# SamSweere/xmm-superres-denoise

Measured on NVIDIA B200. Metric: RRDB SR-2x inference images/sec (F=32, nb=4, 416x416 -> 832x832, batch 64 per GPU), higher is better.
Workload: dtype bf16

## Files before the change

xmm_superres_denoise_b200/csrc/conv3x3_rdb.cuh:

```cuda
#pragma once
#include <cstdio>

#include "conv3x3_tc.cuh"

namespace xmm {

constexpr int kRdbP = 63;
constexpr int kRdbBoxPx = kRdbP + 2;
constexpr int kRdbTileData = 2 * kRdbBoxPx * 64;
constexpr int kRdbTileBytes = 17 * 512;
constexpr int kRdbThreads = 512;
constexpr int kRdbSlots = 5;
constexpr int kRdbSlotCols = kRdbSlots * 32;
constexpr int kRdbMaxRing = 8;
constexpr int kRdbMaxStages = 16;
template <bool PAIR>
constexpr int kRdbLRing = PAIR ? kRdbMaxStages : 8;
constexpr int kRdbTapBytes = 32 * 64;
constexpr int kRdbGroupBytes = 3 * kRdbTapBytes;
constexpr int kRdbProfSlots = 24;

struct RdbLayerArgs {
  const void* wblob;
  uint32_t w_bytes;
  uint32_t smem_off;
  float lrelu_slope;
  int store;
  __nv_bfloat16* out;
  int out_ctot, out_coff;
};

struct RdbArgs {
  RdbLayerArgs layer[3];
  int cin_off;
  int batch, height, width, band_h, tiles_x;
  long long total_rows;
  int stages, ring0, ring1;
  uint32_t w_total;
  float s0, s1, s2;
  const __nv_bfloat16* r1;
  int r1_ctot, r1_coff;
  const __nv_bfloat16* r2;
  int r2_ctot, r2_coff;
  int backoff_ns;
  int prefetch_rows;
  int split_producers;
  long long* prof;
};

template <int NL>
__host__ __device__ inline int rdb_tile_origin(int t) {
  return t == 0 ? 0 : (kRdbP - (NL - 1)) + (t - 1) * (kRdbP - 2 * (NL - 1));
}
template <int NL>
__host__ __device__ inline int rdb_tiles_x(int width) {
  int n = 1;
  while ((n == 1 ? 0 : rdb_tile_origin<NL>(n - 1) - (NL - 1)) + kRdbP < width) ++n;
  return n;
}

struct RdbPiece {
  int b, x0;
  int own_lo, own_hi;
  int ra, rb;
};

template <int NL, bool PAIR = false>
struct RdbSched {
  int band_h, tiles_x, width, c0, npieces;
  int ncols, rank;
  long long t0, t1;
  __device__ __forceinline__ void init(const RdbArgs& a) {
    band_h = a.band_h;
    tiles_x = a.tiles_x;
    width = a.width;
    if (PAIR) {
      ncols = a.batch * a.tiles_x;
      rank = int(ptx::cluster_ctarank());
      const long long unit = blockIdx.x >> 1, nunits = gridDim.x >> 1;
      t0 = a.total_rows * unit / nunits;
      t1 = a.total_rows * (unit + 1) / nunits;
    } else {
      t0 = a.total_rows * blockIdx.x / gridDim.x;
      t1 = a.total_rows * (blockIdx.x + 1) / gridDim.x;
    }
    c0 = int(t0 / band_h);
    npieces = t1 > t0 ? int((t1 - 1) / band_h) - c0 + 1 : 0;
  }
  __device__ __forceinline__ RdbPiece get(int i) const {
    RdbPiece p;
    int col = c0 + i;
    const long long base = (long long)col * band_h;
    p.ra = t0 > base ? int(t0 - base) : 0;
    p.rb = t1 < base + band_h ? int(t1 - base) : band_h;
    bool phantom = false;
    if (PAIR) {
      col = 2 * col + rank;
      phantom = col >= ncols;
      if (phantom) col = ncols - 1;
    }
    p.b = col / tiles_x;
    const int t = col - p.b * tiles_x;
    p.own_lo = rdb_tile_origin<NL>(t);
    p.x0 = t == 0 ? 0 : p.own_lo - (NL - 1);
    p.own_hi = phantom ? p.own_lo : t == tiles_x - 1 ? width : rdb_tile_origin<NL>(t + 1);
    return p;
  }
};

template <int NL, class S, class F>
__device__ __forceinline__ void rdb_walk(const S& s, F&& f) {
  int piece[NL], r[NL], hi[NL], n[NL], seq[NL][NL];
  RdbPiece pc[NL];
  bool done[NL];
#pragma unroll
  for (int l = 0; l < NL; ++l) {
    piece[l] = 0;
    n[l] = 0;
    done[l] = s.npieces == 0;
#pragma unroll
    for (int m = 0; m < NL; ++m) seq[l][m] = 0;
    pc[l] = s.get(0);
    r[l] = pc[l].ra - (NL - 1 - l) - 1;
    hi[l] = pc[l].rb + (NL - 1 - l) + 2;
  }
  while (!done[NL - 1]) {
    uint32_t go = done[0] ? 0u : 1u;
    bool steady = !done[0];
    int reps = pc[0].rb + (NL - 1) - r[0] + 1;
#pragma unroll
    for (int l = 1; l < NL; ++l) {
      const bool ready = !done[l] && (done[l - 1] || piece[l - 1] > piece[l] || (piece[l - 1] == piece[l] && r[l - 1] > r[l] + 1));
      go |= ready ? (1u << l) : 0u;
      steady = steady && ready && piece[l] == piece[0];
      const int kl = pc[l].rb + (NL - 1 - l) - r[l] + 1;
      reps = kl < reps ? kl : reps;
    }
    if (!steady || reps < 1) reps = 1;
    for (int i = 0; i < reps; ++i) {
#pragma unroll
      for (int l = 0; l < NL; ++l) {
        if ((go >> l) & 1u) {
          const int e = NL - 1 - l;
          f(l, pc[l], r[l], r[l] > pc[l].rb + e, n[l], seq[l]);
          ++n[l];
          if (++r[l] > hi[l]) {
#pragma unroll
            for (int m = 0; m < NL; ++m) seq[l][m] += (pc[l].rb - pc[l].ra) + 2 * (NL - 1 - m);
            if (++piece[l] >= s.npieces) {
              done[l] = true;
            } else {
              pc[l] = s.get(piece[l]);
              r[l] = pc[l].ra - e - 1;
              hi[l] = pc[l].rb + e + 2;
            }
          }
        }
      }
    }
  }
}

__device__ __noinline__ void rdb_wait_timeout(int tag, int a, int b2, int c) {
  printf("conv3x3_rdb: CTA %d thread %d stuck in wait %d (layer/map %d, index %d, parity %d)\n", int(blockIdx.x),
         int(threadIdx.x), tag, a, b2, c);
  __trap();
}
__device__ __forceinline__ void rdb_wait(uint64_t* bar, uint32_t parity, int tag, int a, int b2) {
  uint32_t spins = 0;
  while (!ptx::mbar_try_wait(bar, parity)) {
    if (++spins > (1u << 26)) rdb_wait_timeout(tag, a, b2, int(parity));
  }
}

__device__ __forceinline__ void rdb_wait_backoff(uint64_t* bar, uint32_t parity, int tag, int a, int b2, uint32_t ns) {
  uint32_t spins = 0;
  while (!ptx::mbar_try_wait(bar, parity)) {
    if (ns) __nanosleep(ns);
    if (++spins > (1u << 24)) rdb_wait_timeout(tag, a, b2, int(parity));
  }
}
#ifndef XMM_RDB_PROFILE
#define XMM_RDB_PROFILE 0
#endif
__device__ __forceinline__ void rdb_wait_p(uint64_t* bar, uint32_t parity, int tag, int a, int b2, bool prof, long long& acc) {
  if (XMM_RDB_PROFILE && prof) {
    const long long t0 = clock64();
    rdb_wait(bar, parity, tag, a, b2);
    acc += clock64() - t0;
  } else {
    rdb_wait(bar, parity, tag, a, b2);
  }
}

__device__ __forceinline__ int rdb_phi(int row) { return (row + 30) % 3; }

__device__ __forceinline__ void tmem_st_zero32(uint32_t taddr) {
  const uint32_t z = 0;
  asm volatile(
      "tcgen05.st.sync.aligned.32x32b.x32.b32 [%0], "
      "{%1, %1, %1, %1, %1, %1, %1, %1, %1, %1, %1, %1, %1, %1, %1, %1, "
      "%1, %1, %1, %1, %1, %1, %1, %1, %1, %1, %1, %1, %1, %1, %1, %1};" ::"r"(taddr),
      "r"(z)
      : "memory");
}
__device__ __forceinline__ void tmem_st_32x32(uint32_t taddr, const uint32_t (&r)[32]) {
  asm volatile(
      "tcgen05.st.sync.aligned.32x32b.x32.b32 [%0], "
      "{%1, %2, %3, %4, %5, %6, %7, %8, %9, %10, %11, %12, %13, %14, %15, %16, "
      "%17, %18, %19, %20, %21, %22, %23, %24, %25, %26, %27, %28, %29, %30, %31, %32};" ::"r"(taddr),
      "r"(r[0]), "r"(r[1]), "r"(r[2]), "r"(r[3]), "r"(r[4]), "r"(r[5]), "r"(r[6]), "r"(r[7]), "r"(r[8]), "r"(r[9]), "r"(r[10]),
      "r"(r[11]), "r"(r[12]), "r"(r[13]), "r"(r[14]), "r"(r[15]), "r"(r[16]), "r"(r[17]), "r"(r[18]), "r"(r[19]), "r"(r[20]),
      "r"(r[21]), "r"(r[22]), "r"(r[23]), "r"(r[24]), "r"(r[25]), "r"(r[26]), "r"(r[27]), "r"(r[28]), "r"(r[29]), "r"(r[30]),
      "r"(r[31])
      : "memory");
}
__device__ __forceinline__ void st_global_256(void* p, const uint4& a, const uint4& b) {
  asm volatile("st.global.v8.b32 [%0], {%1, %2, %3, %4, %5, %6, %7, %8};" ::"l"(p), "r"(a.x), "r"(a.y), "r"(a.z), "r"(a.w),
               "r"(b.x), "r"(b.y), "r"(b.z), "r"(b.w)
               : "memory");
}
__device__ __forceinline__ void ld_global_nc_256(const void* p, uint4& a, uint4& b) {
  asm volatile("ld.global.nc.v8.b32 {%0, %1, %2, %3, %4, %5, %6, %7}, [%8];"
               : "=r"(a.x), "=r"(a.y), "=r"(a.z), "=r"(a.w), "=r"(b.x), "=r"(b.y), "=r"(b.z), "=r"(b.w)
               : "l"(p));
}
__device__ __forceinline__ void tmem_st_wait() { asm volatile("tcgen05.wait::st.sync.aligned;" ::: "memory"); }

struct RdbCtx {
  uint8_t* w_s;
  uint8_t* stage_s;
  uint8_t* map_s[2];
  uint64_t* lfull;
  uint64_t* empty;
  uint64_t* tfull;
  uint64_t* tdrain;
  uint64_t* mfull;
  uint64_t* mempty;
  uint64_t* w_bar;
  volatile int* lstage;
  uint32_t tmem_base;
};

template <int G, int NL, int L, bool PAIR>
__device__ __forceinline__ void rdb_issuer(const RdbArgs& args, const RdbCtx& c, const RdbSched<NL, PAIR>& sched) {
  constexpr int NM = NL - 1;
  constexpr int e = NL - 1 - L;
  constexpr int ring[2] = {NL == 3 ? 5 : 2, 3};
  constexpr uint32_t kR = kRdbLRing<PAIR>;
  rdb_wait(c.w_bar, 0, 7, L, 0);
  ptx::tc_fence_after();
  const uint64_t bdesc0 = ptx::umma_smem_desc(ptx::smem_u32(c.w_s), 16, 512, ptx::UMMA_SW64);
  const uint64_t adesc0 = ptx::umma_smem_desc(ptx::smem_u32(c.stage_s), 16, 512, ptx::UMMA_SW64);
  const uint32_t a_hi = uint32_t(adesc0 >> 32), b_hi = uint32_t(bdesc0 >> 32);
  const uint32_t a_lo0 = uint32_t(adesc0);
  const uint32_t b_l = uint32_t(bdesc0) + (args.layer[L].smem_off >> 4);
  const uint32_t a_map0[2] = {a_lo0 + uint32_t((c.map_s[0] - c.stage_s) >> 4), a_lo0 + uint32_t((c.map_s[1] - c.stage_s) >> 4)};
  constexpr uint32_t kTile16 = uint32_t(kRdbTileBytes) >> 4;
  constexpr uint32_t kGroup16 = uint32_t(PAIR ? kRdbGroupBytes / 2 : kRdbGroupBytes) >> 4;
  constexpr uint32_t kChunk16 = 3 * kGroup16;
  constexpr uint32_t kIdesc = ptx::umma_idesc_bf16_f32(PAIR ? 256 : 128, 96, 0, 0);
  auto issue6 = [&](uint32_t d, uint32_t a, uint32_t b) {
#pragma unroll
    for (int dx = 0; dx < 3; ++dx)
#pragma unroll
      for (int ks = 0; ks < 2; ++ks) {
        const uint32_t a_lo = a + uint32_t((dx * 64 + ks * 32) >> 4), b_lo = b + uint32_t(dx) * kGroup16 + uint32_t((ks * 32) >> 4);
        if constexpr (PAIR)
          ptx::umma_ss_lh_pair<true>(d, a_lo, a_hi, b_lo, b_hi, kIdesc);
        else
          ptx::umma_ss_lh<true>(d, a_lo, a_hi, b_lo, b_hi, kIdesc);
      }
  };
  auto commit = [](uint64_t* bar) {
    if constexpr (PAIR)
      ptx::umma_commit_pair(bar);
    else
      ptx::umma_commit(bar);
  };
  const bool prof = XMM_RDB_PROFILE && args.prof != nullptr && L == 0;
  long long pw[3] = {0, 0, 0};
  const long long t_begin = XMM_RDB_PROFILE ? clock64() : 0;
  uint32_t fills = 0;
  uint32_t n = 0;
  int seq[2] = {0, 0};
  for (int pi = 0; pi < sched.npieces; ++pi) {
    const RdbPiece pc = sched.get(pi);
    const int r_last = pc.rb + e;
    for (int r = pc.ra - e - 1; r <= r_last + 2; ++r, ++n) {
      if (n > 0) rdb_wait_p(&c.tdrain[L], (n - 1u) & 1u, 2, L, int(n), prof, pw[0]);
      ptx::tc_fence_after();
      if (r <= r_last) {
        const uint32_t d = c.tmem_base + uint32_t(L * kRdbSlotCols + rdb_phi(r - 1) * 32);
        auto global_chunks = [&]() {
#pragma unroll
          for (int g = 0; g < G; ++g) {
            const int k = int(fills % kR);
            rdb_wait_p(&c.lfull[L * kR + k], (fills / kR) & 1u, 3, L, k, prof, pw[1]);
            const int stage = c.lstage[L * kR + k];
            ++fills;
            ptx::tc_fence_after();
            issue6(d, a_lo0 + uint32_t(stage) * kTile16, b_l + uint32_t(g) * kChunk16);
            commit(&c.empty[stage]);
          }
        };
        auto map_chunks = [&]() {
#pragma unroll
          for (int m = 0; m < NM; ++m)
            if (m < L) {
              const int sq = seq[m] + (r - (pc.ra - (NL - 1 - m)));
              const int slot = sq % ring[m];
              rdb_wait_p(&c.mfull[m * 8 + slot], uint32_t(sq / ring[m]) & 1u, 4, L * 10 + m, sq, prof, pw[2]);
              ptx::tc_fence_after();
              issue6(d, a_map0[m] + uint32_t(slot) * kTile16, b_l + uint32_t(G + m) * kChunk16);
              if (L == NL - 1 || r < pc.ra - e || r > pc.rb + e - 1) commit(&c.mempty[m * 8 + slot]);
            }
        };
        if (NL == 2) {
          map_chunks();
          global_chunks();
        } else {
          global_chunks();
          map_chunks();
        }
      }
      commit(&c.tfull[L]);
    }
#pragma unroll
    for (int m = 0; m < NM; ++m) seq[m] += (pc.rb - pc.ra) + 2 * (NL - 1 - m);
  }
  if (XMM_RDB_PROFILE && prof) {
    long long* o = args.prof + size_t(blockIdx.x) * kRdbProfSlots;
    o[0] = clock64() - t_begin;
    o[1] = pw[0];
    o[2] = pw[1];
    o[3] = pw[2];
  }
}

template <int G, int NL, int L, bool PAIR>
__device__ __forceinline__ void rdb_epilogue(const RdbArgs& args, const RdbCtx& c, const RdbSched<NL, PAIR>& sched, int q,
                                             int lane) {
  const bool remote = PAIR && sched.rank != 0;
  auto arrive = [&](uint64_t* bar) {
    if (remote)
      ptx::mbar_arrive_cluster(ptx::mapa(ptx::smem_u32(bar), 0));
    else
      ptx::mbar_arrive(bar);
  };
  constexpr int e = NL - 1 - L;
  constexpr int ring[2] = {NL == 3 ? 5 : 2, 3};
  constexpr bool last = L == NL - 1;
  const int pos = q * 32 + lane + 1;
  const int band = pos >= kRdbBoxPx ? 1 : 0;
  const int pl = band ? pos - (kRdbBoxPx + 1) : pos - 1;
  const bool lane_ok = band ? pl >= 0 : pl < kRdbP;
  const uint32_t lane_base = c.tmem_base + (uint32_t(q * 32) << 16) + uint32_t(L * kRdbSlotCols);
  const uint32_t pos_off = uint32_t(pos) * 64u;
  const uint32_t pos_xor = uint32_t(pos >> 1) & 3u;
  const uint32_t bias_a = ptx::smem_u32(c.w_s + args.layer[L].smem_off + args.layer[L].w_bytes);
  const float slope = args.layer[L].lrelu_slope;
  const bool has_r1 = last && args.r1 != nullptr, has_r2 = last && args.r2 != nullptr;
  const bool prof = XMM_RDB_PROFILE && args.prof != nullptr;
  long long pw[2] = {0, 0};
  long long ph[4] = {0, 0, 0, 0};
  long long tph = 0;
  const long long t_begin = XMM_RDB_PROFILE ? clock64() : 0;
  uint32_t n = 0;
  int seq = 0;
  for (int pi = 0; pi < sched.npieces; ++pi) {
    const RdbPiece pc = sched.get(pi);
    const int px = pc.x0 + pl;
    const bool px_ok = lane_ok && px < args.width;
    const bool px_own = px_ok && px >= pc.own_lo && px < pc.own_hi;
    for (int r = pc.ra - e - 1; r <= pc.rb + e + 2; ++r, ++n) {
      const int j = r - 1;
      const bool real = j >= pc.ra - e && j < pc.rb + e;
      const int y = band * args.band_h + j;
      const bool inimg = px_ok && y >= 0 && y < args.height;
      const bool owned = real && px_own && inimg && j >= pc.ra && j < pc.rb;
      const size_t pix = size_t((pc.b * args.height + (y < 0 ? 0 : y)) * args.width + (px_ok ? px : 0));
      uint4 res1[4], res2[4];
      if (has_r1 && owned) {
        const __nv_bfloat16* p = args.r1 + pix * args.r1_ctot + args.r1_coff;
        ld_global_nc_256(p, res1[0], res1[1]);
        ld_global_nc_256(p + 16, res1[2], res1[3]);
      }
      if (has_r2 && owned) {
        const __nv_bfloat16* p = args.r2 + pix * args.r2_ctot + args.r2_coff;
        ld_global_nc_256(p, res2[0], res2[1]);
        ld_global_nc_256(p + 16, res2[2], res2[3]);
      }
      if (XMM_RDB_PROFILE)
        rdb_wait_p(&c.tfull[L], n & 1u, 5, L, int(n), prof, pw[0]);
      else
        rdb_wait_backoff(&c.tfull[L], n & 1u, 5, L, int(n), uint32_t(args.backoff_ns));
      if (XMM_RDB_PROFILE) tph = clock64();
      ptx::tc_fence_after();
      const int phi = rdb_phi(j);
      const uint32_t t_main = lane_base + uint32_t(phi * 32);
      const uint32_t t_carry = lane_base + uint32_t((3 + phi) * 32);
      float v[32];
      {
        uint32_t accr[32];
        ptx::tmem_ld_32x32(t_main, accr);
        if (phi < 2) {
          uint32_t car[32];
          ptx::tmem_ld_32x32(t_carry, car);
          ptx::tmem_ld_wait();
#pragma unroll
          for (int k = 0; k < 32; ++k) v[k] = __uint_as_float(car[k]) + __uint_as_float(accr[k]);
          tmem_st_zero32(t_carry);
        } else {
          ptx::tmem_ld_wait();
#pragma unroll
          for (int k = 0; k < 32; ++k) v[k] = __uint_as_float(accr[k]);
        }
      }
      {
        uint32_t b32[32];
#pragma unroll
        for (int k = 0; k < 8; ++k)
          asm volatile("ld.shared.v4.u32 {%0, %1, %2, %3}, [%4];"
                       : "=r"(b32[4 * k]), "=r"(b32[4 * k + 1]), "=r"(b32[4 * k + 2]), "=r"(b32[4 * k + 3])
                       : "r"(bias_a + 16u * k));
        tmem_st_32x32(t_main, b32);
      }
      tmem_st_wait();
      ptx::tc_fence_before();
      __syncwarp();
      if (lane == 0) arrive(&c.tdrain[L]);
      if (XMM_RDB_PROFILE) {
        const long long t = clock64();
        ph[0] += t - tph;
        tph = t;
      }
      if (!real) continue;

      if (slope != 1.f) {
#pragma unroll
        for (int k = 0; k < 32; ++k) v[k] = fmaxf(v[k], v[k] * slope);
      }
      if (last) {
        const float s0 = args.s0;
        if (s0 != 1.f) {
#pragma unroll
          for (int k = 0; k < 32; ++k) v[k] *= s0;
        }
        if (has_r1 && owned) {
          const float s1 = args.s1;
#pragma unroll
          for (int k = 0; k < 4; ++k) {
            float m8[8];
            unpack8(res1[k], m8);
#pragma unroll
            for (int i = 0; i < 8; ++i) v[8 * k + i] = fmaf(s1, m8[i], v[8 * k + i]);
          }
        }
        if (has_r2 && owned) {
          const float s2 = args.s2;
#pragma unroll
          for (int k = 0; k < 4; ++k) {
            float m8[8];
            unpack8(res2[k], m8);
#pragma unroll
            for (int i = 0; i < 8; ++i) v[8 * k + i] = fmaf(s2, m8[i], v[8 * k + i]);
          }
        }
      }
      uint4 o[4];
#pragma unroll
      for (int k = 0; k < 4; ++k) o[k] = pack8(v + 8 * k);
      if (XMM_RDB_PROFILE) {
        const long long t = clock64();
        ph[1] += t - tph;
        tph = t;
      }
      if (args.layer[L].store && owned) {
        __nv_bfloat16* gp = args.layer[L].out + pix * args.layer[L].out_ctot + args.layer[L].out_coff;
        st_global_256(gp, o[0], o[1]);
        st_global_256(gp + 16, o[2], o[3]);
      }
      if (!last) {
        const int sq = seq + (j - (pc.ra - e));
        const int slot = sq % ring[L];
        rdb_wait_p(&c.mempty[L * 8 + slot], (uint32_t(sq / ring[L]) & 1u) ^ 1u, 6, L, sq, prof, pw[1]);
        if (XMM_RDB_PROFILE) tph = clock64();
        uint8_t* dst = c.map_s[L] + size_t(slot) * kRdbTileBytes + pos_off;
        const uint4 zero = make_uint4(0, 0, 0, 0);
#pragma unroll
        for (int k = 0; k < 4; ++k) *reinterpret_cast<uint4*>(dst + ((uint32_t(k) ^ pos_xor) << 4)) = inimg ? o[k] : zero;
        ptx::fence_proxy_async();
        __syncwarp();
        if (lane == 0) arrive(&c.mfull[L * 8 + slot]);
        if (XMM_RDB_PROFILE) {
          const long long t = clock64();
          ph[2] += t - tph;
          tph = t;
        }
      }
      if (XMM_RDB_PROFILE) {
        const long long t = clock64();
        ph[3] += t - tph;
        tph = t;
      }
    }
    seq += (pc.rb - pc.ra) + 2 * e;
  }
  if (XMM_RDB_PROFILE && prof && q == 0 && lane == 0 && L < 2) {
    long long* o = args.prof + size_t(blockIdx.x) * kRdbProfSlots + 4 + 4 * L;
    o[0] = clock64() - t_begin;
    o[1] = pw[0];
    o[2] = pw[1];
    o[3] = (long long)n;
    long long* o2 = args.prof + size_t(blockIdx.x) * kRdbProfSlots + 12 + 4 * L;
    o2[0] = ph[0];
    o2[1] = ph[1];
    o2[2] = ph[2];
    o2[3] = ph[3];
  }
}

template <int G, int NL, int L>
__device__ __forceinline__ void rdb_layer_producer(const CUtensorMap* tmap_in, const RdbArgs& args, const RdbCtx& c,
                                                   const RdbSched<NL>& sched, int s0, int ns) {
  constexpr int e = NL - 1 - L;
  int idx = 0;
  uint32_t phase = 0;
  uint32_t fills = 0;
  for (int pi = 0; pi < sched.npieces; ++pi) {
    const RdbPiece pc = sched.get(pi);
    for (int r = pc.ra - e - 1; r <= pc.rb + e; ++r) {
      int row = r, band0 = 0;
      if (r < 0) {
        row = r + args.band_h;
        band0 = -1;
      } else if (r >= args.band_h) {
        row = r - args.band_h;
        band0 = 1;
      }
#pragma unroll
      for (int g = 0; g < G; ++g) {
        const int stage = s0 + idx;
        rdb_wait_backoff(&c.empty[stage], phase ^ 1u, 1, L, stage, uint32_t(args.backoff_ns));
        const int k = int(fills++ & 7u);
        c.lstage[L * 8 + k] = stage;
        uint64_t* fb = &c.lfull[L * 8 + k];
        ptx::mbar_expect_tx(fb, kRdbTileData);
        ptx::tma_load_5d(c.stage_s + size_t(stage) * kRdbTileBytes, tmap_in, fb, args.cin_off + 32 * g, pc.x0 - 1, row, band0, pc.b);
        if (++idx == ns) {
          idx = 0;
          phase ^= 1u;
        }
      }
      if (L == 0 && args.prefetch_rows > 0) {
        const int rp = r + args.prefetch_rows;
        if (rp <= pc.rb + e) {
          int prow = rp, pband = 0;
          if (rp < 0) {
            prow = rp + args.band_h;
            pband = -1;
          } else if (rp >= args.band_h) {
            prow = rp - args.band_h;
            pband = 1;
          }
#pragma unroll
          for (int g = 0; g < G; ++g)
            asm volatile("cp.async.bulk.prefetch.tensor.5d.L2.global.tile [%0, {%1, %2, %3, %4, %5}];" ::"l"(
                             reinterpret_cast<uint64_t>(tmap_in)),
                         "r"(args.cin_off + 32 * g), "r"(pc.x0 - 1), "r"(prow), "r"(pband), "r"(pc.b)
                         : "memory");
        }
      }
    }
  }
}

template <int G, int NL, bool PAIR = false>
__global__ void __launch_bounds__(kRdbThreads, 1)
conv3x3_rdb_kernel(const __grid_constant__ CUtensorMap tmap_in, const RdbArgs args) {
  static_assert(NL == 2 || NL == 3, "two or three fused layers");
  static_assert(NL * kRdbSlotCols <= 512, "accumulators exceed TMEM");
  constexpr int NM = NL - 1;
  constexpr int kR = kRdbLRing<PAIR>;
  static_assert((3 * kR + kR + 3 + 3 + 16 + 16 + 1) * 8 + 3 * kR * 4 + 4 <= 1024, "barrier block exceeds 1024 B");
  extern __shared__ uint8_t smem_raw[];
  uint8_t* smem = reinterpret_cast<uint8_t*>((reinterpret_cast<uintptr_t>(smem_raw) + 1023) & ~uintptr_t(1023));
  RdbCtx c;
  c.w_s = smem;
  c.stage_s = smem + args.w_total;
  c.map_s[0] = c.stage_s + size_t(args.stages) * kRdbTileBytes;
  c.map_s[1] = c.map_s[0] + size_t(args.ring0) * kRdbTileBytes;
  uint8_t* after = c.map_s[1] + size_t(NM > 1 ? args.ring1 : 0) * kRdbTileBytes;
  uint64_t* bars = reinterpret_cast<uint64_t*>(after);
  c.lfull = bars;
  c.empty = c.lfull + 3 * kR;
  c.tfull = c.empty + kR;
  c.tdrain = c.tfull + 3;
  c.mfull = c.tdrain + 3;
  c.mempty = c.mfull + 16;
  c.w_bar = c.mempty + 16;
  c.lstage = reinterpret_cast<volatile int*>(c.w_bar + 1);
  uint32_t* tmem_ptr_s = reinterpret_cast<uint32_t*>(const_cast<int*>(c.lstage) + 3 * kR);

  const int warp = threadIdx.x >> 5;
  const int lane = threadIdx.x & 31;
  const uint32_t rank = PAIR ? ptx::cluster_ctarank() : 0u;

  if (warp == 0 && lane == 0) {
    ptx::prefetch_tmap(&tmap_in);
    for (int s = 0; s < NL * kR; ++s) ptx::mbar_init(&c.lfull[s], 1);
    for (int s = 0; s < args.stages; ++s) ptx::mbar_init(&c.empty[s], 1);
    for (int l = 0; l < NL; ++l) {
      ptx::mbar_init(&c.tfull[l], 1);
      ptx::mbar_init(&c.tdrain[l], PAIR ? 8 : 4);
    }
    for (int s = 0; s < 16; ++s) {
      ptx::mbar_init(&c.mfull[s], PAIR ? 8 : 4);
      ptx::mbar_init(&c.mempty[s], 1);
    }
    ptx::mbar_init(c.w_bar, 1);
    ptx::fence_mbar_init();
  }
  if (warp == 1) {
    if constexpr (PAIR)
      ptx::tmem_alloc_pair<512>(tmem_ptr_s);
    else
      ptx::tmem_alloc<512>(tmem_ptr_s);
  }
  ptx::tc_fence_before();
  if constexpr (PAIR)
    ptx::cluster_sync();
  else
    __syncthreads();
  ptx::tc_fence_after();
  c.tmem_base = *tmem_ptr_s;

  if (warp == 0 && ptx::elect_one()) {
    uint32_t wtot = 0;
    for (int l = 0; l < NL; ++l) wtot += args.layer[l].w_bytes + 128u;
    ptx::mbar_expect_tx(c.w_bar, wtot);
    for (int l = 0; l < NL; ++l) {
      const uint8_t* gsrc = static_cast<const uint8_t*>(args.layer[l].wblob);
      uint8_t* dst = c.w_s + args.layer[l].smem_off;
      const uint32_t wb = args.layer[l].w_bytes;
      if constexpr (PAIR) {
        constexpr uint32_t kHalf = kRdbGroupBytes / 2;
        for (uint32_t grp = 0; grp < wb / kHalf; ++grp)
          ptx::bulk_load(dst + grp * kHalf, gsrc + grp * kRdbGroupBytes + rank * kHalf, kHalf, c.w_bar);
        ptx::bulk_load(dst + wb, gsrc + 2 * wb, 128u, c.w_bar);
      } else {
        const uint32_t n_l = wb + 128u;
        for (uint32_t off = 0; off < n_l; off += 32768u)
          ptx::bulk_load(dst + off, gsrc + off, n_l - off < 32768u ? n_l - off : 32768u, c.w_bar);
      }
    }
  }
  const int egroup = (warp - 4) >> 2;
  if (warp >= 4) {
    uint4* z = reinterpret_cast<uint4*>(c.map_s[0]);
    const int nz = (args.ring0 + (NM > 1 ? args.ring1 : 0)) * (kRdbTileBytes / 16);
    for (int i = int(threadIdx.x) - 128; i < nz; i += kRdbThreads - 128) z[i] = make_uint4(0, 0, 0, 0);
    ptx::fence_proxy_async();
    if (egroup < NL) {
      rdb_wait(c.w_bar, 0, 9, 0, 0);
      const uint32_t lane_base = c.tmem_base + (uint32_t((warp & 3) * 32) << 16) + uint32_t(egroup * kRdbSlotCols);
      const float* bias_s = reinterpret_cast<const float*>(c.w_s + args.layer[egroup].smem_off + args.layer[egroup].w_bytes);
      uint32_t b32[32];
#pragma unroll
      for (int k = 0; k < 32; ++k) b32[k] = __float_as_uint(bias_s[k]);
      for (int sl = 0; sl < 3; ++sl) tmem_st_32x32(lane_base + uint32_t(sl * 32), b32);
      for (int sl = 3; sl < kRdbSlots; ++sl) tmem_st_zero32(lane_base + uint32_t(sl * 32));
      tmem_st_wait();
    }
  }
  ptx::tc_fence_before();
  if constexpr (PAIR)
    ptx::cluster_sync();
  else
    __syncthreads();
  ptx::tc_fence_after();

  RdbSched<NL, PAIR> sched;
  sched.init(args);

  if (!PAIR && NL == 2 && args.split_producers && (warp == 0 || warp == 3)) {
    if constexpr (!PAIR) {
      if (ptx::elect_one()) {
        const int ns0 = (args.stages + 1) / 2;
        if (warp == 0) rdb_layer_producer<G, NL, 0>(&tmap_in, args, c, sched, 0, ns0);
        if (warp == 3) rdb_layer_producer<G, NL, 1>(&tmap_in, args, c, sched, ns0, args.stages - ns0);
      }
    }
  } else if (warp == 0) {
    if (ptx::elect_one()) {
      int stage = 0;
      uint32_t phase = 0;
      uint32_t fills[NL];
#pragma unroll
      for (int l = 0; l < NL; ++l) fills[l] = 0;
      rdb_walk<NL>(sched, [&](int l, const RdbPiece& pc, int r, bool flush, int, const int*) {
        if (flush) return;
        int row = r, band0 = 0;
        if (r < 0) {
          row = r + args.band_h;
          band0 = -1;
        } else if (r >= args.band_h) {
          row = r - args.band_h;
          band0 = 1;
        }
#pragma unroll
        for (int g = 0; g < G; ++g) {
          rdb_wait_backoff(&c.empty[stage], phase ^ 1u, 1, l, stage, uint32_t(args.backoff_ns));
          const int k = int(fills[l]++ % uint32_t(kR));
          c.lstage[l * kR + k] = stage;
          uint64_t* fb = &c.lfull[l * kR + k];
          if constexpr (PAIR) {
            if (rank == 0) ptx::mbar_expect_tx(fb, 2 * kRdbTileData);
            ptx::tma_load_5d_pair(c.stage_s + size_t(stage) * kRdbTileBytes, &tmap_in, ptx::mapa(ptx::smem_u32(fb), 0),
                                  args.cin_off + 32 * g, pc.x0 - 1, row, band0, pc.b);
          } else {
            ptx::mbar_expect_tx(fb, kRdbTileData);
            ptx::tma_load_5d(c.stage_s + size_t(stage) * kRdbTileBytes, &tmap_in, fb, args.cin_off + 32 * g, pc.x0 - 1, row,
                             band0, pc.b);
          }
          if (++stage == args.stages) {
            stage = 0;
            phase ^= 1u;
          }
        }
        if (l == 0 && args.prefetch_rows > 0) {
          const int rp = r + args.prefetch_rows;
          if (rp <= pc.rb + (NL - 1)) {
            int prow = rp, pband = 0;
            if (rp < 0) {
              prow = rp + args.band_h;
              pband = -1;
            } else if (rp >= args.band_h) {
              prow = rp - args.band_h;
              pband = 1;
            }
#pragma unroll
            for (int g = 0; g < G; ++g)
              asm volatile("cp.async.bulk.prefetch.tensor.5d.L2.global.tile [%0, {%1, %2, %3, %4, %5}];" ::"l"(
                               reinterpret_cast<uint64_t>(&tmap_in)),
                           "r"(args.cin_off + 32 * g), "r"(pc.x0 - 1), "r"(prow), "r"(pband), "r"(pc.b)
                           : "memory");
          }
        }
      });
    }
  } else if (warp <= 3) {
    if (warp - 1 < NL && rank == 0 && ptx::elect_one()) {
      if (warp == 1) rdb_issuer<G, NL, 0, PAIR>(args, c, sched);
      if (warp == 2) rdb_issuer<G, NL, 1, PAIR>(args, c, sched);
      if constexpr (NL == 3) {
        if (warp == 3) rdb_issuer<G, NL, 2, PAIR>(args, c, sched);
      }
    }
  } else if (egroup < NL) {
    const int q = warp & 3;
    if (egroup == 0) rdb_epilogue<G, NL, 0, PAIR>(args, c, sched, q, lane);
    if (egroup == 1) rdb_epilogue<G, NL, 1, PAIR>(args, c, sched, q, lane);
    if constexpr (NL == 3) {
      if (egroup == 2) rdb_epilogue<G, NL, 2, PAIR>(args, c, sched, q, lane);
    }
  }

  ptx::tc_fence_before();
  if constexpr (PAIR)
    ptx::cluster_sync();
  else
    __syncthreads();
  if (warp == 1) {
    ptx::tc_fence_after();
    if constexpr (PAIR)
      ptx::tmem_dealloc_pair<512>(c.tmem_base);
    else
      ptx::tmem_dealloc<512>(c.tmem_base);
  }
}

}
```

xmm_superres_denoise_b200/csrc/xmm_b200.cu:

```cuda
#include "../../include/xmm_b200.h"

#include <unordered_map>
#include <vector>

#include "conv3x3_chain.cuh"
#include "conv3x3_dx.cuh"
#include "conv3x3_row.cuh"
#include "conv3x3_rdb.cuh"
#include "conv3x3_tc.cuh"
#include "edge_kernels.cuh"
#include "host_common.cuh"
#include "loss_kernels.cuh"
#include "pack_weights.cuh"
#include "wgrad_tc.cuh"

#ifndef XMM_DEFAULT_TAP_MODE
#define XMM_DEFAULT_TAP_MODE 0
#endif

using namespace xmm;

extern "C" const char* xmm_last_error(void) { return last_error_ref().c_str(); }
extern "C" int xmm_version(void) { return 100; }
extern "C" int xmm_check_device(void) {
// ... 573 lines not shown
  }
  for (int l = n - 1; used < grid; l = (l + n - 1) % n) { ++cnt[l]; ++used; }
  for (int l = 0; used > grid; l = (l + 1) % n) if (cnt[l] > 1) { --cnt[l]; --used; }
  if (const char* e = getenv("XMM_CHAIN_SPLIT")) {
    int v[kChainMaxLayers], k = 0, sum = 0;
    for (const char* q = e; *q && k < n; ++k) {
      v[k] = atoi(q);
      sum += v[k];
      while (*q && *q != ',') ++q;
      if (*q == ',') ++q;
    }
    if (k == n && sum <= grid) {
      bool ok = true;
      for (int l = 0; l < n; ++l) ok = ok && v[l] >= 1;
      if (ok) for (int l = 0; l < n; ++l) cnt[l] = v[l];
    }
  }
  size_t smem = 0;
  int begin = 0;
  for (int l = 0; l < n; ++l) {
    ChainLayer& c = a.layer[l];
    c.wblob = L[l].wblob;
    c.nchunks = L[l].cin / 32;
    c.w_bytes = uint32_t(c.nchunks) * 9u * Cfg::kTapBytes;
    c.cin_off = L[l].in_coff;
    c.cta_begin = begin;
    c.cta_count = cnt[l];
    begin += cnt[l];
    const size_t fixed = Cfg::smem_bytes(c.w_bytes, 0);
    int stages = int((size_t(dev.max_smem_optin) - fixed) / Cfg::kStageBytes);
    if (stages > kMaxStages) stages = kMaxStages;
    c.stages = stages;
    const size_t need = Cfg::smem_bytes(c.w_bytes, stages);
    if (need > smem) smem = need;
    fill_epilogue(c.epi, L[l]);
    int rc = cached_tmap(&tm.m[l], L[l].in, a.batch, a.height, a.width, L[l].in_ctot, 32, kDxTileW, kDxPatchH);
    if (rc != XMM_OK) return rc;
    rc = cached_tmap(&tm.out[l], L[l].out, a.batch, a.height, a.width, L[l].out_ctot, Cfg::kWarpCols, kDxTileW, 2);
    if (rc != XMM_OK) return rc;
  }
  const int total_ctas = begin;
  XMM_CUDA_OK(cudaMemsetAsync(done, 0, size_t(n) * nstrips * sizeof(int), stream));
  {
    const int rc_attr = ensure_max_smem(reinterpret_cast<const void*>(conv3x3_chain_kernel<32, 32>), dev);
    if (rc_attr != XMM_OK) return rc_attr;
  }
  static const bool prof_on = env_int("XMM_CHAIN_PROF", 0) != 0;
  long long* prof_d = nullptr;
  if (prof_on) {
    XMM_CUDA_OK(cudaMalloc(&prof_d, size_t(total_ctas) * 4 * sizeof(long long)));
    XMM_CUDA_OK(cudaMemsetAsync(prof_d, 0, size_t(total_ctas) * 4 * sizeof(long long), stream));
    a.prof = prof_d;
  }
  void* kargs[2] = {&tm, &a};
  XMM_CUDA_OK(cudaLaunchCooperativeKernel(reinterpret_cast<const void*>(conv3x3_chain_kernel<32, 32>), dim3(total_ctas),
                                          dim3(kDxThreads), kargs, smem, stream));
  if (prof_on) {
    XMM_CUDA_OK(cudaStreamSynchronize(stream));
    std::vector<long long> h(size_t(total_ctas) * 4);
    XMM_CUDA_OK(cudaMemcpy(h.data(), prof_d, h.size() * sizeof(long long), cudaMemcpyDeviceToHost));
    cudaFree(prof_d);
    for (int l = 0; l < n; ++l) {
      double tot = 0, dep = 0, idle = 0, tiles = 0;
      for (int c = a.layer[l].cta_begin; c < a.layer[l].cta_begin + a.layer[l].cta_count; ++c) {
        tot += double(h[size_t(c) * 4]); dep += double(h[size_t(c) * 4 + 1]);
        idle += double(h[size_t(c) * 4 + 2]); tiles += double(h[size_t(c) * 4 + 3]);
      }
      const double nc = a.layer[l].cta_count;
      fprintf(stderr, "chain layer %d: %3d CTAs, nchunks %d, stages %d | per CTA: total %.0f cyc, dependency wait %.0f, "
              "epilogue idle %.0f, tiles %.1f -> %.0f cyc/tile all-in, %.0f cyc/tile busy\n", l, a.layer[l].cta_count,
              a.layer[l].nchunks, a.layer[l].stages, tot / nc, dep / nc, idle / nc, tiles / nc, tot / tiles,
              (tot - idle) / tiles);
    }
  }
  return XMM_OK;
}

}

extern "C" size_t xmm_conv3x3_chain_workspace_bytes(int nlayers, int batch, int height) {
  if (nlayers < 1 || batch < 1 || height < 1) return 0;
  return size_t(nlayers) * size_t(batch) * size_t((height + kDxTileH - 1) / kDxTileH) * sizeof(int);
}

const char* rdb_blocker(const xmm_conv3x3_params* L, int n, const DeviceInfo& dev) {
  if (n != 5) return "five layers";
  const xmm_conv3x3_params& p0 = L[0];
  if (p0.height < 8 || (p0.height & 1)) return "image height must be even (two bands) and >= 8";
  for (int k = 0; k < 5; ++k) {
    const xmm_conv3x3_params& p = L[k];
    if (p.kc != 32 || p.cout != 32) return "kc = cout = 32 layers only";
    if (p.pixel_shuffle != 0 || p.mask != nullptr || p.colsum != nullptr) return "no pixel shuffle / mask / column sums";
    if (p.wblob_row == nullptr) return "no row-hop weight image (wblob_row)";
    if (p.tap_mode > 0) return "a kernel form is forced (tap_mode)";
    if (p.batch != p0.batch || p.height != p0.height || p.width != p0.width) return "one image geometry";
    if (p.in != p0.in || p.in_ctot != p0.in_ctot || p.in_coff != p0.in_coff || p.cin != 32 * (k + 1))
      return "layer k must read channels [c0, c0 + 32 (k+1)) of one buffer";
    if (k < 4) {
      if (p.out != p0.in || p.out_ctot != p0.in_ctot || p.out_coff != p0.in_coff + 32 * (k + 1))
        return "layer k < 5 must write channels [c0 + 32 k, c0 + 32 (k+1)) of the same buffer";
      if (p.r1 != nullptr || p.r2 != nullptr || p.s0 != 1.0f) return "residuals only on the last layer";
    } else {
      if (p.out == p0.in && p.out_coff < p0.in_coff + 160 && p.out_coff + 32 > p0.in_coff)
        return "the last layer may not overwrite the block's own feature maps";
    }
  }
  if ((long long)p0.batch * p0.height * p0.width >= (1LL << 31)) return "more than 2^31 pixels";
  if (size_t(dev.max_smem_optin) < 232448) return "needs 227 KB of shared memory per CTA";
  return nullptr;
}

template <int G, int NL, bool PAIR>
int launch_rdb(const xmm_conv3x3_params* L, const bool* store, const DeviceInfo& dev, cudaStream_t stream) {
  RdbArgs a{};
  uint32_t off = 0;
  for (int l = 0; l < NL; ++l) {
    const xmm_conv3x3_params& p = L[l];
    a.layer[l].wblob = p.wblob_row;
    a.layer[l].w_bytes = uint32_t(p.cin / 32) * 9u * uint32_t(kRdbTapBytes) / (PAIR ? 2u : 1u);
    a.layer[l].smem_off = off;
    off += (a.layer[l].w_bytes + 128u + 1023u) & ~1023u;
    a.layer[l].lrelu_slope = p.lrelu_slope;
    a.layer[l].store = store[l] ? 1 : 0;
    a.layer[l].out = static_cast<__nv_bfloat16*>(p.out);
    a.layer[l].out_ctot = p.out_ctot;
    a.layer[l].out_coff = p.out_coff;
  }
  a.w_total = off;
  const xmm_conv3x3_params& pl = L[NL - 1];
  a.cin_off = L[0].in_coff;
  a.batch = L[0].batch;
  a.height = L[0].height;
  a.width = L[0].width;
  a.band_h = a.height / 2;
  a.tiles_x = rdb_tiles_x<NL>(a.width);
  const long long ncols = (long long)a.batch * a.tiles_x;
  a.total_rows = (PAIR ? (ncols + 1) / 2 : ncols) * a.band_h;
  a.s0 = pl.s0; a.s1 = pl.s1; a.s2 = pl.s2;
  a.r1 = static_cast<const __nv_bfloat16*>(pl.r1); a.r1_ctot = pl.r1_ctot; a.r1_coff = pl.r1_coff;
  a.r2 = static_cast<const __nv_bfloat16*>(pl.r2); a.r2_ctot = pl.r2_ctot; a.r2_coff = pl.r2_coff;
  static const int backoff_env = env_int("XMM_RDB_BACKOFF_NS", 0);
  static const int prefetch_env = env_int("XMM_RDB_PREFETCH_ROWS", 3);
  a.backoff_ns = backoff_env;
  a.prefetch_rows = prefetch_env;
  constexpr int kBarBytes = 1024;
  const long long room = (long long)dev.max_smem_optin - 1024 - kBarBytes - (long long)a.w_total;
  int tiles = int(room / kRdbTileBytes);
  a.ring0 = NL == 3 ? 5 : 2;
  a.ring1 = NL == 3 ? 3 : 0;
  a.stages = tiles - a.ring0 - a.ring1;
  if (a.stages > kRdbLRing<PAIR>) a.stages = kRdbLRing<PAIR>;
  static const int stages_env = env_int("XMM_RDB_STAGES", 0);
  if (stages_env > 0 && stages_env < a.stages) a.stages = stages_env;
  if (a.stages < 3) return fail(XMM_ERR_UNSUPPORTED_SHAPE, "conv3x3 (fused dense block): %d pipeline stages fit", a.stages);
  static const int split_env = env_int("XMM_RDB_SPLIT_PRODUCERS", 0);
  a.split_producers = (!PAIR && NL == 2 && split_env && a.stages >= 4) ? 1 : 0;
  CUtensorMap tmap;
  int rc = cached_band_tmap(&tmap, L[0].in, a.batch, a.height, a.width, L[0].in_ctot, a.band_h, 2, 32, kRdbBoxPx, 2);
  if (rc != XMM_OK) return rc;
  const void* kernel = reinterpret_cast<const void*>(conv3x3_rdb_kernel<G, NL, PAIR>);
  rc = ensure_max_smem(kernel, dev);
  if (rc != XMM_OK) return rc;
  const size_t smem = 1024 + size_t(a.w_total) + size_t(a.stages + a.ring0 + a.ring1) * kRdbTileBytes + kBarBytes;
  static const int max_ctas = env_int("XMM_RDB_MAX_CTAS", 0);
  cudaLaunchConfig_t cfg{};
  cudaLaunchAttribute attr[1];
  cfg.blockDim = dim3(kRdbThreads);
  cfg.dynamicSmemBytes = smem;
  cfg.stream = stream;
  long long grid;
  if constexpr (PAIR) {
    attr[0].id = cudaLaunchAttributeClusterDimension;
    attr[0].val.clusterDim.x = 2;
    attr[0].val.clusterDim.y = 1;
    attr[0].val.clusterDim.z = 1;
    cfg.attrs = attr;
    cfg.numAttrs = 1;
    static int max_clusters = 0;
    if (max_clusters == 0) {
      cfg.gridDim = dim3(unsigned(2 * dev.sm_count));
      XMM_CUDA_OK(cudaOccupancyMaxActiveClusters(&max_clusters, conv3x3_rdb_kernel<G, NL, PAIR>, &cfg));
      if (max_clusters < 1) return fail(XMM_ERR_UNSUPPORTED_SHAPE, "conv3x3 (fused dense block): no CTA pair fits an SM pair");
    }
    long long pairs = a.total_rows < max_clusters ? a.total_rows : max_clusters;
    if (max_ctas > 0 && pairs > max_ctas / 2) pairs = max_ctas / 2 > 0 ? max_ctas / 2 : 1;
    grid = 2 * pairs;
  } else {
    grid = a.total_rows < dev.sm_count ? a.total_rows : dev.sm_count;
    if (max_ctas > 0 && grid > max_ctas) grid = max_ctas;
  }
  cfg.gridDim = dim3(unsigned(grid));
  static const int prof_env = XMM_RDB_PROFILE ? env_int("XMM_RDB_PROF", 0) : 0;
  static long long* prof_dev = nullptr;
  constexpr size_t kProfBytes = kRdbProfSlots * sizeof(long long) * 1024;
  if (prof_env) {
    if (prof_dev == nullptr) XMM_CUDA_OK(cudaMalloc(&prof_dev, kProfBytes));
    XMM_CUDA_OK(cudaMemsetAsync(prof_dev, 0, kProfBytes, stream));
    a.prof = prof_dev;
  }
  if constexpr (PAIR) {
    XMM_CUDA_OK(cudaLaunchKernelEx(&cfg, conv3x3_rdb_kernel<G, NL, PAIR>, tmap, a));
  } else {
    conv3x3_rdb_kernel<G, NL, PAIR><<<cfg.gridDim, kRdbThreads, smem, stream>>>(tmap, a);
    XMM_CUDA_OK(cudaGetLastError());
  }
  if (prof_env) {
    XMM_CUDA_OK(cudaStreamSynchronize(stream));
    std::vector<long long> h(size_t(grid) * kRdbProfSlots);
    XMM_CUDA_OK(cudaMemcpy(h.data(), prof_dev, h.size() * sizeof(long long), cudaMemcpyDeviceToHost));
    static const char* names[kRdbProfSlots] = {
        "issuer total", "issuer wait drained", "issuer wait TMA", "issuer wait map row",
        "epi0 total", "epi0 wait row complete", "epi0 wait map slot", "epi0 rows",
        "epi1 total", "epi1 wait row complete", "epi1 wait map slot", "epi1 rows",
        "epi0 drain (ld+st+arrive)", "epi0 math+pack", "epi0 map write+fence+arrive", "epi0 global store",
        "epi1 drain (ld+st+arrive)", "epi1 math+residuals+pack", "epi1 map write (none)", "epi1 global store",
        "", "", "", ""};
    fprintf(stderr, "conv3x3_rdb<%d,%d%s> grid %lld stages %d:", G, NL, PAIR ? ",pair" : "", grid, a.stages);
    for (int k = 0; k < 20; ++k) {
      double sum = 0;
      int n = 0;
      for (long long c = 0; c < grid; ++c)
        if (k >= 4 || !PAIR || c % 2 == 0) {
          sum += double(h[size_t(c) * kRdbProfSlots + k]);
          ++n;
        }
      fprintf(stderr, " %s %.0f;", names[k], sum / n);
    }
    fprintf(stderr, "\n");
  }
  return XMM_OK;
}

bool rdb_pair(int mode_flags) {
  if (mode_flags & XMM_CHAIN_RDB_PAIR) return true;
  if (mode_flags & XMM_CHAIN_RDB_SINGLE) return false;
  static const int pair_env = env_int("XMM_RDB_PAIR", 1);
  return pair_env != 0;
}

int launch_rdb_block(const xmm_conv3x3_params* L, bool skip_dead, bool pair, const DeviceInfo& dev, cudaStream_t stream) {
  const bool store_a[3] = {true, true, true};
  int rc = launch_rdb<1, 3, false>(L, store_a, dev, stream);
  if (rc != XMM_OK) return rc;
  const bool store_b[2] = {!skip_dead, true};
  return pair ? launch_rdb<4, 2, true>(L + 3, store_b, dev, stream) : launch_rdb<4, 2, false>(L + 3, store_b, dev, stream);
}

extern "C" int xmm_set_sm_reserve(int sms) {
  if (sms < 0) sms = 0;
  return sm_reserve().exchange(sms);
}

namespace {
thread_local int g_last_chain_launches = 0;
}
extern "C" int xmm_last_chain_launches(void) { return g_last_chain_launches; }

extern "C" int xmm_conv3x3_chain_bf16(const xmm_conv3x3_params* layers, int nlayers, int mode_flags, void* workspace,
                                      size_t workspace_bytes, void* stream) {
  XMM_REQUIRE(layers != nullptr && nlayers >= 1, "conv3x3_chain: no layers");
  g_last_chain_launches = 0;
  const int mode = mode_flags & 0xff;
  const bool skip_dead = (mode_flags & XMM_CHAIN_SKIP_DEAD_STORES) != 0;
  constexpr int kFlags = XMM_CHAIN_SKIP_DEAD_STORES | XMM_CHAIN_RDB_PAIR | XMM_CHAIN_RDB_SINGLE;
  XMM_REQUIRE(mode >= 0 && mode <= 3 && (mode_flags & ~(0xff | kFlags)) == 0 &&
                  (mode_flags & (XMM_CHAIN_RDB_PAIR | XMM_CHAIN_RDB_SINGLE)) != (XMM_CHAIN_RDB_PAIR | XMM_CHAIN_RDB_SINGLE),
              "conv3x3_chain: mode must be 0 (auto), 1 (pipelined), 2 (layer by layer) or 3 (fused dense block), with at most "
              "one of the pair / single flags");
  DeviceInfo dev;
  int rc = require_sm100(&dev);
  if (rc != XMM_OK) return rc;
  for (int l = 0; l < nlayers; ++l) {
    rc = check_conv_params(layers[l]);
    if (rc != XMM_OK) return rc;
  }
  cudaStream_t s = static_cast<cudaStream_t>(stream);
  static const int rdb_env = env_int("XMM_RDB", 1);
  if (mode == 3 || (mode == 0 && rdb_env)) {
    const char* why_not = rdb_blocker(layers, nlayers, dev);
    if (why_not == nullptr) {
      g_last_chain_launches = 2;
      return launch_rdb_block(layers, skip_dead, rdb_pair(mode_flags), dev, s);
    }
    if (mode == 3) return fail(XMM_ERR_UNSUPPORTED_SHAPE, "conv3x3_chain: cannot fuse the dense block (%s)", why_not);
  }
  const char* why = chain_blocker(layers, nlayers);
  bool pipelined = mode == 1 && why == nullptr;
  if (mode == 1 && why != nullptr) return fail(XMM_ERR_UNSUPPORTED_SHAPE, "conv3x3_chain: cannot pipeline (%s)", why);
  if (pipelined) {
    const size_t need = xmm_conv3x3_chain_workspace_bytes(nlayers, layers[0].batch, layers[0].height);
    XMM_REQUIRE(workspace != nullptr && workspace_bytes >= need && (reinterpret_cast<uintptr_t>(workspace) & 3) == 0,
                "conv3x3_chain: workspace of %zu bytes needed (got %zu)", need, workspace_bytes);
    g_last_chain_launches = 1;
    return launch_chain(layers, nlayers, dev, static_cast<int*>(workspace), s);
  }
  for (int l = 0; l < nlayers; ++l) {
    rc = xmm_conv3x3_bf16(&layers[l], stream);
    if (rc != XMM_OK) return rc;
  }
  g_last_chain_launches = nlayers;
  return XMM_OK;
}

extern "C" int xmm_normalize(const xmm_normalize_params* pp, void* stream) {
  XMM_REQUIRE(pp != nullptr, "normalize: null params");
  const xmm_normalize_params& p = *pp;
  DeviceInfo dev;
  int rc = require_sm100(&dev);
  if (rc != XMM_OK) return rc;
  if (p.n == 0) return XMM_OK;
  XMM_REQUIRE(p.in && p.out, "normalize: null tensor pointer");
  XMM_REQUIRE(p.stretch_mode >= 0 && p.stretch_mode <= 3, "normalize: Stretching function %d is not implemented",
              p.stretch_mode);
  XMM_REQUIRE((reinterpret_cast<uintptr_t>(p.in) & 15) == 0 && (reinterpret_cast<uintptr_t>(p.out) & 15) == 0,
              "normalize: pointers must be 16-byte aligned");
  XMM_REQUIRE(!p.mask || p.mask_n > 0, "normalize: mask_n must be > 0 with a mask");
  cudaStream_t s = static_cast<cudaStream_t>(stream);
  NormalizeArgs a{};
  a.in = p.in; a.mask = p.mask; a.out = p.out; a.n = p.n; a.mask_n = p.mask_n; a.in_is_int32 = p.in_is_int32;
  a.pre_scale = p.pre_scale; a.max_val = p.max_val; a.mode = p.stretch_mode; a.dyn_max = p.scratch;
  if (!(p.max_val > 0.0f)) {
    XMM_REQUIRE(p.scratch != nullptr && !p.in_is_int32 && p.mask == nullptr,
                "normalize: the max_val <= 0 branch needs fp32 input, no mask and a scratch float");
    XMM_CUDA_OK(cudaMemsetAsync(p.scratch, 0, sizeof(float), s));
    max_kernel<<<dev.sm_count * 4, 256, 0, s>>>(static_cast<const float*>(p.in), p.n, p.pre_scale, p.scratch);
    XMM_CUDA_OK(cudaGetLastError());
  }
  const size_t threads = (p.n + 3) / 4;
  normalize_kernel<<<unsigned((threads + 255) / 256), 256, 0, s>>>(a);
  XMM_CUDA_OK(cudaGetLastError());
  return XMM_OK;
}

extern "C" int xmm_denormalize(const float* in, float* out, size_t n, size_t per_image, const float* max_vals_dev,
                               int max_n, int stretch_mode, void* stream) {
  DeviceInfo dev;
  int rc = require_sm100(&dev);
  if (rc != XMM_OK) return rc;
  if (n == 0) return XMM_OK;
  XMM_REQUIRE(in && out && max_vals_dev, "denormalize: null tensor pointer");
  XMM_REQUIRE(stretch_mode >= 0 && stretch_mode <= 3, "denormalize: Stretching function %d is not implemented",
              stretch_mode);
  XMM_REQUIRE(max_n == 1 || (per_image > 0 && size_t(max_n) * per_image == n),
              "denormalize: %d max values do not match %zu elements of %zu per image", max_n, n, per_image);
  denormalize_kernel<<<unsigned((n + 255) / 256), 256, 0, static_cast<cudaStream_t>(stream)>>>(
      in, out, n, per_image ? per_image : n, max_vals_dev, max_n, stretch_mode);
  XMM_CUDA_OK(cudaGetLastError());
  return XMM_OK;
}

extern "C" int xmm_restretch(const float* in, float* out, size_t n, int from_mode, int to_mode, void* stream) {
  DeviceInfo dev;
  int rc = require_sm100(&dev);
  if (rc != XMM_OK) return rc;
  if (n == 0) return XMM_OK;
  XMM_REQUIRE(in && out, "restretch: null tensor pointer");
  XMM_REQUIRE(from_mode >= 0 && from_mode <= 3 && to_mode >= 0 && to_mode <= 3,
              "restretch: Stretching function %d -> %d is not implemented", from_mode, to_mode);
  XMM_REQUIRE((reinterpret_cast<uintptr_t>(in) & 15) == 0 && (reinterpret_cast<uintptr_t>(out) & 15) == 0,
              "restretch: pointers must be 16-byte aligned");
  const size_t threads = (n + 3) / 4;
  restretch_kernel<<<unsigned((threads + 255) / 256), 256, 0, static_cast<cudaStream_t>(stream)>>>(in, out, n, from_mode,
                                                                                                  to_mode);
  XMM_CUDA_OK(cudaGetLastError());
  return XMM_OK;
}

extern "C" int xmm_prepare_counts(const xmm_prepare_counts_params* pp, void* stream) {
  XMM_REQUIRE(pp != nullptr, "prepare_counts: null params");
  const xmm_prepare_counts_params& p = *pp;
  DeviceInfo dev;
  int rc = require_sm100(&dev);
  if (rc != XMM_OK) return rc;
  XMM_REQUIRE(p.nsrc >= 1 && p.nsrc <= 3 && p.src[0] && p.out, "prepare_counts: 1..3 source planes and an output");
  for (int k = 0; k < p.nsrc; ++k) XMM_REQUIRE(p.src[k] != nullptr, "prepare_counts: source plane %d is null", k);
  XMM_REQUIRE(p.batch > 0 && p.h > 0 && p.w > 0 && p.res_h > 0 && p.res_w > 0 && p.up >= 1,
              "prepare_counts: bad shape %dx%dx%d (x%d) -> %dx%d", p.batch, p.h, p.w, p.up, p.res_h, p.res_w);
  XMM_REQUIRE(p.max_val > 0.0f, "prepare_counts: max_val must be positive");
  XMM_REQUIRE(p.stretch_mode >= 0 && p.stretch_mode <= 3, "prepare_counts: Stretching function %d is not implemented",
              p.stretch_mode);
  PrepareCountsArgs a{};
  for (int k = 0; k < 3; ++k) a.src[k] = k < p.nsrc ? p.src[k] : nullptr;
  a.nsrc = p.nsrc; a.src_is_int32 = p.src_is_int32; a.mask = p.mask;
  a.batch = p.batch; a.h = p.h; a.w = p.w; a.up = p.up; a.res_h = p.res_h; a.res_w = p.res_w;
  a.pre_scale = p.pre_scale; a.pre_scale_dev = p.pre_scale_dev; a.max_val = p.max_val; a.mode = p.stretch_mode;
  a.out = p.out;
  const size_t n = size_t(p.batch) * p.res_h * p.res_w;
  prepare_counts_kernel<<<unsigned((n + 255) / 256), 256, 0, static_cast<cudaStream_t>(stream)>>>(a);
  XMM_CUDA_OK(cudaGetLastError());
  return XMM_OK;
}

extern "C" int xmm_image_upsample(const float* in, float* out, int n_img, int h, int w, int scale, void* stream) {
  DeviceInfo dev;
  int rc = require_sm100(&dev);
  if (rc != XMM_OK) return rc;
  XMM_REQUIRE(scale >= 1, "image_upsample: scale factor %d must be a positive integer", scale);
  const size_t n_out = size_t(n_img) * h * w * scale * scale;
// ... 449 lines not shown
```

Measured before the change: 1439.

## Run first RDB kernel as CTA pair with shared input ring across layers

Enables the CTA-pair (2-SM cluster) path for the three-layer G=1 dense-block kernel by default. For that kernel it replaces the per-layer load rings with a single shared x0 ring that one producer fills once per row. All three layers consume the same staged tile, and only the last consumer releases the slot. This is meant to remove redundant TMA loads of the same input rows for each fused layer and to use paired MMA. In exchange, slot lifetime grows, so stall risk rises and at least four stages are required.

Result: faster. 1497 (median of 6 runs) (+4.0%).

```diff
diff --git a/xmm_superres_denoise_b200/csrc/conv3x3_rdb.cuh b/xmm_superres_denoise_b200/csrc/conv3x3_rdb.cuh
--- a/xmm_superres_denoise_b200/csrc/conv3x3_rdb.cuh
+++ b/xmm_superres_denoise_b200/csrc/conv3x3_rdb.cuh
@@ -16,6 +16,8 @@
 constexpr int kRdbMaxStages = 16;
 template <bool PAIR>
 constexpr int kRdbLRing = PAIR ? kRdbMaxStages : 8;
+template <int G, bool PAIR>
+constexpr bool kRdbXRing = PAIR && G == 1;
 constexpr int kRdbTapBytes = 32 * 64;
 constexpr int kRdbGroupBytes = 3 * kRdbTapBytes;
 constexpr int kRdbProfSlots = 24;
@@ -284,6 +286,7 @@
   uint32_t fills = 0;
   uint32_t n = 0;
   int seq[2] = {0, 0};
+  int xseq = 0;
   for (int pi = 0; pi < sched.npieces; ++pi) {
     const RdbPiece pc = sched.get(pi);
     const int r_last = pc.rb + e;
@@ -293,15 +296,32 @@
       if (r <= r_last) {
         const uint32_t d = c.tmem_base + uint32_t(L * kRdbSlotCols + rdb_phi(r - 1) * 32);
         auto global_chunks = [&]() {
-#pragma unroll
-          for (int g = 0; g < G; ++g) {
-            const int k = int(fills % kR);
-            rdb_wait_p(&c.lfull[L * kR + k], (fills / kR) & 1u, 3, L, k, prof, pw[1]);
-            const int stage = c.lstage[L * kR + k];
-            ++fills;
+          if constexpr (kRdbXRing<G, PAIR>) {
+            if (L > 0 && r == pc.ra - e - 1) {
+#pragma unroll
+              for (int m = 0; m < NM; ++m)
+                if (m < L) {
+                  const int sq = seq[m] + (r - (pc.ra - (NL - 1 - m)));
+                  rdb_wait_p(&c.mfull[m * 8 + sq % ring[m]], uint32_t(sq / ring[m]) & 1u, 4, L * 10 + m, sq, prof, pw[2]);
+                }
+            }
+            const int sq = xseq + (r - (pc.ra - NL));
+            const int slot = sq % args.stages;
+            rdb_wait_p(&c.lfull[slot], uint32_t(sq / args.stages) & 1u, 3, L, sq, prof, pw[1]);
             ptx::tc_fence_after();
-            issue6(d, a_lo0 + uint32_t(stage) * kTile16, b_l + uint32_t(g) * kChunk16);
-            commit(&c.empty[stage]);
+            issue6(d, a_lo0 + uint32_t(slot) * kTile16, b_l);
+            if (L == NL - 1 || r < pc.ra - e || r > pc.rb + e - 1) commit(&c.empty[slot]);
+          } else {
+#pragma unroll
+            for (int g = 0; g < G; ++g) {
+              const int k = int(fills % kR);
+              rdb_wait_p(&c.lfull[L * kR + k], (fills / kR) & 1u, 3, L, k, prof, pw[1]);
+              const int stage = c.lstage[L * kR + k];
+              ++fills;
+              ptx::tc_fence_after();
+              issue6(d, a_lo0 + uint32_t(stage) * kTile16, b_l + uint32_t(g) * kChunk16);
+              commit(&c.empty[stage]);
+            }
           }
         };
         auto map_chunks = [&]() {
@@ -328,6 +348,7 @@
     }
 #pragma unroll
     for (int m = 0; m < NM; ++m) seq[m] += (pc.rb - pc.ra) + 2 * (NL - 1 - m);
+    xseq += (pc.rb - pc.ra) + 2 * NL;
   }
   if (XMM_RDB_PROFILE && prof) {
     long long* o = args.prof + size_t(blockIdx.x) * kRdbProfSlots;
@@ -576,6 +597,35 @@
   }
 }
 
+template <int NL>
+__device__ __forceinline__ void rdb_x0_producer(const CUtensorMap* tmap_in, const RdbArgs& args, const RdbCtx& c,
+                                                const RdbSched<NL, true>& sched) {
+  int slot = 0;
+  uint32_t phase = 0;
+  for (int pi = 0; pi < sched.npieces; ++pi) {
+    const RdbPiece pc = sched.get(pi);
+    for (int r = pc.ra - NL; r <= pc.rb + NL - 1; ++r) {
+      int row = r, band0 = 0;
+      if (r < 0) {
+        row = r + args.band_h;
+        band0 = -1;
+      } else if (r >= args.band_h) {
+        row = r - args.band_h;
+        band0 = 1;
+      }
+      rdb_wait_backoff(&c.empty[slot], phase ^ 1u, 1, 0, slot, uint32_t(args.backoff_ns));
+      uint64_t* fb = &c.lfull[slot];
+      if (sched.rank == 0) ptx::mbar_expect_tx(fb, 2 * kRdbTileData);
+      ptx::tma_load_5d_pair(c.stage_s + size_t(slot) * kRdbTileBytes, tmap_in, ptx::mapa(ptx::smem_u32(fb), 0),
+                            args.cin_off, pc.x0 - 1, row, band0, pc.b);
+      if (++slot == args.stages) {
+        slot = 0;
+        phase ^= 1u;
+      }
+    }
+  }
+}
+
 template <int G, int NL, bool PAIR = false>
 __global__ void __launch_bounds__(kRdbThreads, 1)
 conv3x3_rdb_kernel(const __grid_constant__ CUtensorMap tmap_in, const RdbArgs args) {
@@ -583,7 +633,10 @@
   static_assert(NL * kRdbSlotCols <= 512, "accumulators exceed TMEM");
   constexpr int NM = NL - 1;
   constexpr int kR = kRdbLRing<PAIR>;
-  static_assert((3 * kR + kR + 3 + 3 + 16 + 16 + 1) * 8 + 3 * kR * 4 + 4 <= 1024, "barrier block exceeds 1024 B");
+  constexpr bool XR = kRdbXRing<G, PAIR>;
+  constexpr int kFull = XR ? kR : 3 * kR;
+  constexpr int kStageIds = XR ? 0 : 3 * kR;
+  static_assert((kFull + kR + 3 + 3 + 16 + 16 + 1) * 8 + kStageIds * 4 + 4 <= 1024, "barrier block exceeds 1024 B");
   extern __shared__ uint8_t smem_raw[];
   uint8_t* smem = reinterpret_cast<uint8_t*>((reinterpret_cast<uintptr_t>(smem_raw) + 1023) & ~uintptr_t(1023));
   RdbCtx c;
@@ -594,14 +647,14 @@
   uint8_t* after = c.map_s[1] + size_t(NM > 1 ? args.ring1 : 0) * kRdbTileBytes;
   uint64_t* bars = reinterpret_cast<uint64_t*>(after);
   c.lfull = bars;
-  c.empty = c.lfull + 3 * kR;
+  c.empty = c.lfull + kFull;
   c.tfull = c.empty + kR;
   c.tdrain = c.tfull + 3;
   c.mfull = c.tdrain + 3;
   c.mempty = c.mfull + 16;
   c.w_bar = c.mempty + 16;
   c.lstage = reinterpret_cast<volatile int*>(c.w_bar + 1);
-  uint32_t* tmem_ptr_s = reinterpret_cast<uint32_t*>(const_cast<int*>(c.lstage) + 3 * kR);
+  uint32_t* tmem_ptr_s = reinterpret_cast<uint32_t*>(const_cast<int*>(c.lstage) + kStageIds);
 
   const int warp = threadIdx.x >> 5;
   const int lane = threadIdx.x & 31;
@@ -609,7 +662,7 @@
 
   if (warp == 0 && lane == 0) {
     ptx::prefetch_tmap(&tmap_in);
-    for (int s = 0; s < NL * kR; ++s) ptx::mbar_init(&c.lfull[s], 1);
+    for (int s = 0; s < (XR ? kFull : NL * kR); ++s) ptx::mbar_init(&c.lfull[s], 1);
     for (int s = 0; s < args.stages; ++s) ptx::mbar_init(&c.empty[s], 1);
     for (int l = 0; l < NL; ++l) {
       ptx::mbar_init(&c.tfull[l], 1);
@@ -692,8 +745,12 @@
         if (warp == 3) rdb_layer_producer<G, NL, 1>(&tmap_in, args, c, sched, ns0, args.stages - ns0);
       }
     }
+  } else if (XR && warp == 0) {
+    if constexpr (XR) {
+      if (ptx::elect_one()) rdb_x0_producer<NL>(&tmap_in, args, c, sched);
+    }
   } else if (warp == 0) {
-    if (ptx::elect_one()) {
+    if (!XR && ptx::elect_one()) {
       int stage = 0;
       uint32_t phase = 0;
       uint32_t fills[NL];
diff --git a/xmm_superres_denoise_b200/csrc/xmm_b200.cu b/xmm_superres_denoise_b200/csrc/xmm_b200.cu
--- a/xmm_superres_denoise_b200/csrc/xmm_b200.cu
+++ b/xmm_superres_denoise_b200/csrc/xmm_b200.cu
@@ -749,7 +749,9 @@
   if (a.stages > kRdbLRing<PAIR>) a.stages = kRdbLRing<PAIR>;
   static const int stages_env = env_int("XMM_RDB_STAGES", 0);
   if (stages_env > 0 && stages_env < a.stages) a.stages = stages_env;
-  if (a.stages < 3) return fail(XMM_ERR_UNSUPPORTED_SHAPE, "conv3x3 (fused dense block): %d pipeline stages fit", a.stages);
+  const int min_stages = kRdbXRing<G, PAIR> ? 4 : 3;
+  if (a.stages < min_stages)
+    return fail(XMM_ERR_UNSUPPORTED_SHAPE, "conv3x3 (fused dense block): %d pipeline stages fit", a.stages);
   static const int split_env = env_int("XMM_RDB_SPLIT_PRODUCERS", 0);
   a.split_producers = (!PAIR && NL == 2 && split_env && a.stages >= 4) ? 1 : 0;
   CUtensorMap tmap;
@@ -828,19 +830,19 @@
   return XMM_OK;
 }
 
-bool rdb_pair(int mode_flags) {
-  if (mode_flags & XMM_CHAIN_RDB_PAIR) return true;
-  if (mode_flags & XMM_CHAIN_RDB_SINGLE) return false;
-  static const int pair_env = env_int("XMM_RDB_PAIR", 1);
-  return pair_env != 0;
-}
-
-int launch_rdb_block(const xmm_conv3x3_params* L, bool skip_dead, bool pair, const DeviceInfo& dev, cudaStream_t stream) {
+int rdb_pair(int mode_flags) {
+  if (mode_flags & XMM_CHAIN_RDB_PAIR) return 3;
+  if (mode_flags & XMM_CHAIN_RDB_SINGLE) return 0;
+  static const int pair_env = env_int("XMM_RDB_PAIR", 3);
+  return pair_env & 3;
+}
+
+int launch_rdb_block(const xmm_conv3x3_params* L, bool skip_dead, int pair, const DeviceInfo& dev, cudaStream_t stream) {
   const bool store_a[3] = {true, true, true};
-  int rc = launch_rdb<1, 3, false>(L, store_a, dev, stream);
+  int rc = (pair & 1) ? launch_rdb<1, 3, true>(L, store_a, dev, stream) : launch_rdb<1, 3, false>(L, store_a, dev, stream);
   if (rc != XMM_OK) return rc;
   const bool store_b[2] = {!skip_dead, true};
-  return pair ? launch_rdb<4, 2, true>(L + 3, store_b, dev, stream) : launch_rdb<4, 2, false>(L + 3, store_b, dev, stream);
+  return (pair & 2) ? launch_rdb<4, 2, true>(L + 3, store_b, dev, stream) : launch_rdb<4, 2, false>(L + 3, store_b, dev, stream);
 }
 
 extern "C" int xmm_set_sm_reserve(int sms) {
```
